# drprojects/superpoint_transformer

Hardware: AMD Instinct MI355X
Metric: Mpoints/s SPT fwd+bwd on S3DIS-scale NAG (higher is better)
Workload: dtype f32 (the reference's shipped matmul class - configs/train.yaml:60-61 `float32_matmul_precision: high` = TF32 / bf16x3 next to `precision: 32` - as bf16x3: matrix products on the bf16 pipe with split operands, attention and the backward of the fused layers and of the attention blocks' Linears hi*hi +

## Files before the change

superpoint_transformer_amd/csrc/fused_mlp.hip:

```cpp
#include <math.h>
#include <stdlib.h>

#include "common.hpp"

namespace spt {
namespace fmlp {

typedef float f32x4 __attribute__((ext_vector_type(4)));
constexpr int WAVES = 4;
constexpr int TR = 16;
constexpr int MAX_BLOCKS = 1024;
constexpr int MAX_BWD_WAVES = 4096;

__device__ __forceinline__ double xg_sum_d(double v) {
  v += __shfl_xor(v, 16, 64);
  v += __shfl_xor(v, 32, 64);
  return v;
}
__device__ __forceinline__ void wave_sync_lds() {
  __builtin_amdgcn_fence(__ATOMIC_RELEASE, "wavefront");
  __builtin_amdgcn_wave_barrier();
  __builtin_amdgcn_fence(__ATOMIC_ACQUIRE, "wavefront");
}

// ... 347 lines not shown
        *reinterpret_cast<float4*>(gl + rr * LDG + n) = v;
      }
    }
    stage_tile<KPP, LDX, KPP>(xprev, row0, cnt, K, false, pt, pslope, xl, nullptr, lane);
    wave_sync_lds();
#pragma unroll
    for (int r = 0; r < 4; ++r) {
      float xb[KB];
#pragma unroll
      for (int kb = 0; kb < KB; ++kb) {
        const int k = 16 * kb + c;
        float v = xl[(4 * g + r) * LDX + k];
        if (pre) {
          v = fmaf(v - pt[k], pt[KPP + k], pt[2 * KPP + k]);
          v = (v > 0.f) ? v : v * pslope;
          v = (4 * g + r < cnt && k < K) ? v : 0.f;
        }
        xb[kb] = v;
      }
#pragma unroll
      for (int nb = 0; nb < NBK; ++nb) {
        const float ga = gl[(4 * g + r) * LDG + 16 * nb + c];
#pragma unroll
        for (int kb = 0; kb < KB; ++kb)
          C3[nb][kb] = __builtin_amdgcn_mfma_f32_16x16x4f32(ga, xb[kb], C3[nb][kb], 0, 0, 0);
      }
    }
    if constexpr (NEED_GX) {
      f32x4 CX[KB];
#pragma unroll
      for (int kb = 0; kb < KB; ++kb) CX[kb] = (f32x4){0.f, 0.f, 0.f, 0.f};
      if constexpr (W_IN_LDS) {
        constexpr int G = (KB > 4) ? 1 : 2;
        float ac[G], bc[G][KB], an[G], bn[G][KB];
#pragma unroll
        for (int u = 0; u < G; ++u) {
          ac[u] = gl[c * LDG + 4 * u + g];
#pragma unroll
          for (int kb = 0; kb < KB; ++kb) bc[u][kb] = w_lds[(4 * u + g) * LDW + 16 * kb + c];
        }
#pragma unroll
        for (int grp = 0; grp < N / 4 / G; ++grp) {
          if (grp + 1 < N / 4 / G) {
#pragma unroll
            for (int u = 0; u < G; ++u) {
              const int st = G * (grp + 1) + u;
              an[u] = gl[c * LDG + 4 * st + g];
#pragma unroll
              for (int kb = 0; kb < KB; ++kb) bn[u][kb] = w_lds[(4 * st + g) * LDW + 16 * kb + c];
            }
          }
          __builtin_amdgcn_sched_barrier(0);
#pragma unroll
          for (int u = 0; u < G; ++u)
#pragma unroll
            for (int kb = 0; kb < KB; ++kb)
              CX[kb] = __builtin_amdgcn_mfma_f32_16x16x4f32(ac[u], bc[u][kb], CX[kb], 0, 0, 0);
          __builtin_amdgcn_sched_barrier(0);
#pragma unroll
          for (int u = 0; u < G; ++u) {
            ac[u] = an[u];
#pragma unroll
            for (int kb = 0; kb < KB; ++kb) bc[u][kb] = bn[u][kb];
          }
        }
      } else {
#pragma unroll
        for (int st = 0; st < N / 4; ++st) {
          const float a = gl[c * LDG + 4 * st + g];
#pragma unroll
          for (int kb = 0; kb < KB; ++kb)
            CX[kb] = __builtin_amdgcn_mfma_f32_16x16x4f32(a, BW[st][kb], CX[kb], 0, 0, 0);
        }
      }
#pragma unroll
      for (int r = 0; r < 4; ++r) {
        const int rr = 4 * g + r;
        if (rr < cnt) {
#pragma unroll
          for (int kb = 0; kb < KB; ++kb) {
            const int k = 16 * kb + c;
            if (k < K) {
              const float v = CX[kb][r];
              gx[(row0 + rr) * K + k] = v;
              if (pre) {
                const float o = xl[rr * LDX + k] - pt[k];
                float gg = v;
                if (pslope != 1.f) {
                  const float y = fmaf(o, pt[KPP + k], pt[2 * KPP + k]);
                  gg = (y > 0.f) ? gg : gg * pslope;
                }
                p1[kb] += (double)gg;
                p2[kb] += (double)gg * (double)o;
              }
            }
          }
        }
      }
    }
  }
  float* gwp = gw_partial + (size_t)wave * N * K;
#pragma unroll
  for (int nb = 0; nb < NBK; ++nb)
#pragma unroll
    for (int kb = 0; kb < KB; ++kb)
#pragma unroll
      for (int r = 0; r < 4; ++r) {
        const int k = 16 * kb + c;
        if (k < K) gwp[(size_t)(16 * nb + 4 * g + r) * K + k] = C3[nb][kb][r];
      }
  if (pstat_partial) {
    double* pp = pstat_partial + (size_t)wave * (2 * K + 1);
#pragma unroll
    for (int kb = 0; kb < KB; ++kb) {
      const double a = xg_sum_d(p1[kb]), b = xg_sum_d(p2[kb]);
      const int k = 16 * kb + c;
      if (g == 0 && k < K) {
        pp[k] = a;
        pp[K + k] = b;
      }
    }
    if (lane == 0) pp[2 * K] = (wave == 0) ? (double)(r1 - r0) : 0.0;
  }
}

typedef __bf16 bf16x8 __attribute__((ext_vector_type(8)));
typedef __bf16 bf16x4 __attribute__((ext_vector_type(4)));
typedef short s16x4 __attribute__((ext_vector_type(4)));

template <int NV, typename V>
__device__ __forceinline__ void split_bf16(const float (&x)[NV], V& hi, V& lo) {
#pragma unroll
  for (int i = 0; i < NV; ++i) {
    const __bf16 h = (__bf16)x[i];
    hi[i] = h;
    lo[i] = (__bf16)(x[i] - (float)h);
  }
}
template <bool LO>
__device__ __forceinline__ f32x4 mfma3_32(const bf16x8& ah, const bf16x8& al, const bf16x8& bh,
                                          const bf16x8& bl, f32x4 c) {
  if constexpr (LO) {
    c = __builtin_amdgcn_mfma_f32_16x16x32_bf16(al, bh, c, 0, 0, 0);
    c = __builtin_amdgcn_mfma_f32_16x16x32_bf16(ah, bl, c, 0, 0, 0);
  }
  return __builtin_amdgcn_mfma_f32_16x16x32_bf16(ah, bh, c, 0, 0, 0);
}
template <bool LO>
__device__ __forceinline__ f32x4 mfma3_16(const bf16x4& ah, const bf16x4& al, const bf16x4& bh,
                                          const bf16x4& bl, f32x4 c) {
  const s16x4 AH = __builtin_bit_cast(s16x4, ah), AL = __builtin_bit_cast(s16x4, al);
  const s16x4 BH = __builtin_bit_cast(s16x4, bh), BL = __builtin_bit_cast(s16x4, bl);
  if constexpr (LO) {
    c = __builtin_amdgcn_mfma_f32_16x16x16bf16_1k(AL, BH, c, 0, 0, 0);
    c = __builtin_amdgcn_mfma_f32_16x16x16bf16_1k(AH, BL, c, 0, 0, 0);
  }
  return __builtin_amdgcn_mfma_f32_16x16x16bf16_1k(AH, BH, c, 0, 0, 0);
}

template <int K4, int NBK, bool LO, bool IN16 = false, bool OUT16 = false>
__global__ __launch_bounds__(WAVES * 64, 2) void fwd_kernel_bf(
    const float* __restrict__ x, int64_t r0, int64_t r1, int K, const float* __restrict__ W,
    const float* __restrict__ am, const float* __restrict__ sc, const float* __restrict__ bs,
    float slope, float* __restrict__ h, double* __restrict__ partial, FmlpRuns rt) {
  constexpr int KP = K4 * 4, KS = (KP + 31) / 32, KP32 = KS * 32, LDA = KP32 + 4, N = NBK * 16;
  SPT_FMLP_RUN_FWD(N)
  __shared__ __attribute__((aligned(16))) float a_lds[WAVES][TR * LDA];
  __shared__ __attribute__((aligned(16))) float tab[3 * KP32];
  __shared__ double red[WAVES][2 * N];
  const int lane = threadIdx.x & 63;
  const int wid = __builtin_amdgcn_readfirstlane(threadIdx.x >> 6);
  const int g = lane >> 4, c = lane & 15;
  float* al = a_lds[wid];
  const bool pre = am != nullptr;
  load_table(tab, am, K, KP32);
  load_table(tab + KP32, sc, K, KP32);
  load_table(tab + 2 * KP32, bs, K, KP32);
  for (int i = lane; i < TR * LDA; i += 64) al[i] = 0.f;
  __syncthreads();

  bf16x8 Bh[NBK][KS], Bl[NBK][KS];
#pragma unroll
  for (int nb = 0; nb < NBK; ++nb)
#pragma unroll
    for (int ks = 0; ks < KS; ++ks) {
      float w[8];
#pragma unroll
      for (int i = 0; i < 8; ++i) {
        const int k = 32 * ks + 8 * g + i;
        w[i] = (k < K) ? W[(size_t)(16 * nb + c) * K + k] : 0.f;
      }
      split_bf16<8>(w, Bh[nb][ks], Bl[nb][ks]);
    }
  double s1[NBK], s2[NBK];
#pragma unroll
  for (int nb = 0; nb < NBK; ++nb) s1[nb] = s2[nb] = 0.0;

  const int64_t ntiles = (r1 - r0 + TR - 1) / TR;
  const int64_t wave = (int64_t)blockIdx.x * WAVES + wid;
  const int64_t nwaves = (int64_t)gridDim.x * WAVES;
  for (int64_t t = wave; t < ntiles; t += nwaves) {
    const int64_t row0 = r0 + t * TR;
    const int cnt = (int)((r1 - row0) < TR ? (r1 - row0) : TR);
    wave_sync_lds();
    stage_tile<KP32, LDA, KP32, false, 4, IN16>(x, row0, cnt, K, pre, tab, slope, al, nullptr, lane);
    wave_sync_lds();
    f32x4 C[NBK];
#pragma unroll
    for (int nb = 0; nb < NBK; ++nb) C[nb] = (f32x4){0.f, 0.f, 0.f, 0.f};
#pragma unroll
    for (int ks = 0; ks < KS; ++ks) {
      const float4 a0 = *reinterpret_cast<const float4*>(al + c * LDA + 32 * ks + 8 * g);
      const float4 a1 = *reinterpret_cast<const float4*>(al + c * LDA + 32 * ks + 8 * g + 4);
      const float av[8] = {a0.x, a0.y, a0.z, a0.w, a1.x, a1.y, a1.z, a1.w};
      bf16x8 ah, alo;
      split_bf16<8>(av, ah, alo);
#pragma unroll
      for (int nb = 0; nb < NBK; ++nb) C[nb] = mfma3_32<LO>(ah, alo, Bh[nb][ks], Bl[nb][ks], C[nb]);
    }
    if constexpr (OUT16) {
      constexpr int ROWB = 2 * N + 16;
      static_assert(TR * ROWB <= TR * LDA * 4, "the packed output tile fits the A-tile buffer");
      static_assert((TR * N / 8) % 64 == 0 || TR * N / 8 < 64, "whole 16-byte chunks");
      wave_sync_lds();
      char* ob = reinterpret_cast<char*>(al);
#pragma unroll
      for (int r = 0; r < 4; ++r) {
        const int rr = 4 * g + r;
#pragma unroll
        for (int nb = 0; nb < NBK; ++nb) {
          const unsigned mine = bf16_bits(C[nb][r]);
          const float vr = __uint_as_float(mine << 16);
          if (rr < cnt) {
            s1[nb] += (double)vr;
            s2[nb] += (double)vr * (double)vr;
          }
          const unsigned other = (unsigned)__builtin_amdgcn_update_dpp(0, (int)mine, 0xB1, 0xF, 0xF, false);
          if ((c & 1) == (r & 1)) {
            const unsigned w = (c & 1) ? (other | (mine << 16)) : (mine | (other << 16));
            *reinterpret_cast<unsigned*>(ob + rr * ROWB + (16 * nb + (c & ~1)) * 2) = w;
          }
        }
      }
      wave_sync_lds();
      constexpr int CPR = N / 8;
      uint16_t* h16 = reinterpret_cast<uint16_t*>(h);
#pragma unroll
      for (int q = lane; q < TR * CPR; q += 64) {
        const int rr = q / CPR, ch = q - rr * CPR;
        if (rr < cnt)
          *reinterpret_cast<uint4*>(h16 + (row0 + rr) * N + ch * 8) =
              *reinterpret_cast<const uint4*>(ob + rr * ROWB + ch * 16);
      }
    } else {
#pragma unroll
      for (int r = 0; r < 4; ++r) {
        const int rr = 4 * g + r;
        if (rr < cnt) {
          float* hr = h + (row0 + rr) * N + c;
#pragma unroll
          for (int nb = 0; nb < NBK; ++nb) {
            const float v = C[nb][r];
            hr[16 * nb] = v;
            s1[nb] += (double)v;
            s2[nb] += (double)v * (double)v;
          }
        }
      }
    }
  }
#pragma unroll
  for (int nb = 0; nb < NBK; ++nb) {
    const double a = xg_sum_d(s1[nb]), b = xg_sum_d(s2[nb]);
    if (g == 0) {
      red[wid][nb * 16 + c] = a;
      red[wid][N + nb * 16 + c] = b;
    }
  }
  __syncthreads();
  double* out = partial + (size_t)blockIdx.x * (2 * N + 1);
  for (int i = threadIdx.x; i < 2 * N; i += WAVES * 64)
    out[i] = ((red[0][i] + red[1][i]) + red[2][i]) + red[3][i];
  if (threadIdx.x == 0) out[2 * N] = (blockIdx.x == 0) ? (double)(r1 - r0) : 0.0;
}

constexpr int WAVES_X3 = 8;
template <int NV, typename V>
__device__ __forceinline__ void split3_bf16(const float (&x)[NV], V& h, V& m, V& l) {
#pragma unroll
  for (int i = 0; i < NV; ++i) {
    const __bf16 a = (__bf16)x[i];
    const float r1 = x[i] - (float)a;
    const __bf16 b = (__bf16)r1;
    const float r2 = r1 - (float)b;
    h[i] = a;
    m[i] = b;
    l[i] = (__bf16)r2;
  }
}
template <int K4, int NBK>
__global__ __launch_bounds__(WAVES_X3 * 64, 2) void fwd_kernel_x3(
    const float* __restrict__ x, int64_t r0, int64_t r1, int K, const float* __restrict__ W,
    const float* __restrict__ am, const float* __restrict__ sc, const float* __restrict__ bs,
    float slope, float* __restrict__ h, double* __restrict__ partial, FmlpRuns rt) {
  constexpr int KP = K4 * 4, KS = (KP + 31) / 32, KP32 = KS * 32, LDA = KP32 + 4, N = NBK * 16;
  constexpr int LDW = KP32 + 8;
  SPT_FMLP_RUN_FWD(N)
  __shared__ __attribute__((aligned(16))) float a_lds[WAVES_X3][TR * LDA];
// ... 1785 lines not shown
```

superpoint_transformer_amd/csrc/fused_mlp_dma.hip:

```cpp
#include <math.h>

#include "common.hpp"

#ifndef SPT_FDMA_SKIP
#define SPT_FDMA_SKIP 0
#endif

namespace spt {
namespace fdma {

typedef float f32x4 __attribute__((ext_vector_type(4)));
typedef __bf16 bf16x8 __attribute__((ext_vector_type(8)));
typedef __bf16 bf16x4 __attribute__((ext_vector_type(4)));
typedef short s16x4 __attribute__((ext_vector_type(4)));
constexpr int TR = 16;

__device__ __forceinline__ double xg_sum_d(double v) {
  v += __shfl_xor(v, 16, 64);
  v += __shfl_xor(v, 32, 64);
  return v;
}
__device__ __forceinline__ void lds_order() {
  __builtin_amdgcn_fence(__ATOMIC_RELEASE, "wavefront");
  __builtin_amdgcn_wave_barrier();
  __builtin_amdgcn_fence(__ATOMIC_ACQUIRE, "wavefront");
}
__device__ __forceinline__ void lds_dma16(const void* g, float* lds) {
#if SPT_FDMA_SKIP & 32
  return;
#endif
  const unsigned a = __builtin_amdgcn_readfirstlane(
      (unsigned)(size_t)((__attribute__((address_space(3))) void*)lds));
  asm volatile("s_mov_b32 m0, %0\n\ts_nop 0\n\tglobal_load_lds_dwordx4 %1, off"
               :: "s"(a), "v"(g) : "memory");
}
__device__ __forceinline__ void lds_dma4(const void* g, float* lds) {
#if SPT_FDMA_SKIP & 32
  return;
#endif
  const unsigned a = __builtin_amdgcn_readfirstlane(
      (unsigned)(size_t)((__attribute__((address_space(3))) void*)lds));
  asm volatile("s_mov_b32 m0, %0\n\ts_nop 0\n\tglobal_load_lds_dword %1, off"
               :: "s"(a), "v"(g) : "memory");
}
__device__ __forceinline__ void wait_vm0() {
  asm volatile("s_waitcnt vmcnt(0)" ::: "memory");
  __builtin_amdgcn_fence(__ATOMIC_ACQUIRE, "wavefront");
}
__device__ __forceinline__ void wait_lds() {
  asm volatile("s_waitcnt lgkmcnt(0)" ::: "memory");
}
__device__ __forceinline__ int opaque(int v) {
  asm volatile("" : "+v"(v));
  return v;
}
template <int NV, typename V>
__device__ __forceinline__ void split_bf16(const float (&x)[NV], V& hi, V& lo) {
#pragma unroll
  for (int i = 0; i < NV; ++i) {
    const __bf16 h = (__bf16)x[i];
    hi[i] = h;
    lo[i] = (__bf16)(x[i] - (float)h);
  }
}
template <bool LO>
__device__ __forceinline__ f32x4 mfma3_32(const bf16x8& ah, const bf16x8& al, const bf16x8& bh,
                                          const bf16x8& bl, f32x4 c) {
  if constexpr (LO) {
    c = __builtin_amdgcn_mfma_f32_16x16x32_bf16(al, bh, c, 0, 0, 0);
    c = __builtin_amdgcn_mfma_f32_16x16x32_bf16(ah, bl, c, 0, 0, 0);
  }
  return __builtin_amdgcn_mfma_f32_16x16x32_bf16(ah, bh, c, 0, 0, 0);
}
template <bool LO>
__device__ __forceinline__ f32x4 mfma3_16(const bf16x4& ah, const bf16x4& al, const bf16x4& bh,
                                          const bf16x4& bl, f32x4 c) {
  const s16x4 AH = __builtin_bit_cast(s16x4, ah), AL = __builtin_bit_cast(s16x4, al);
  const s16x4 BH = __builtin_bit_cast(s16x4, bh), BL = __builtin_bit_cast(s16x4, bl);
  if constexpr (LO) {
    c = __builtin_amdgcn_mfma_f32_16x16x16bf16_1k(AL, BH, c, 0, 0, 0);
    c = __builtin_amdgcn_mfma_f32_16x16x16bf16_1k(AH, BL, c, 0, 0, 0);
  }
  return __builtin_amdgcn_mfma_f32_16x16x16bf16_1k(AH, BH, c, 0, 0, 0);
}

template <int R>
__device__ __forceinline__ int pick_lane(int v, int base, int sel) {
  int r = __builtin_amdgcn_readlane(v, base);
#pragma unroll
  for (int j = 1; j < R; ++j) r = (sel == j) ? __builtin_amdgcn_readlane(v, base + j) : r;
  return r;
}

constexpr int fold_len(int K, int K0) { return (K + (K0 + 16) / 16 * 16) * ((K0 + 16) / 16 * 16); }
template <int K, int N, int NW, int OCC, bool LO, bool POOLED, bool S16 = false, int FK0 = 0>
__global__ __launch_bounds__(NW * 64, OCC) void bwd_dma_kernel(
    const float* __restrict__ gy, const float* __restrict__ h, int64_t r0, int64_t r1,
    const float* __restrict__ am, const float* __restrict__ sc, const float* __restrict__ bs,
    float slope, const float* __restrict__ c1, const float* __restrict__ c2,
    const float* __restrict__ c3, const float* __restrict__ xprev,
    const float* __restrict__ pam, const float* __restrict__ psc, const float* __restrict__ pbs,
    float pslope, const float* __restrict__ W, float* __restrict__ gx,
    float* __restrict__ gw_partial, double* __restrict__ pstat_partial,
    const int32_t* __restrict__ perm, const int32_t* __restrict__ pos_seg,
    const float* __restrict__ gout, const int32_t* __restrict__ arg, FmlpRuns rt,
    const float* __restrict__ x0 = nullptr, const float* __restrict__ fshift = nullptr,
    float* __restrict__ fold_partial = nullptr) {
  constexpr bool FOLD = FK0 > 0;
  constexpr int FOLD_K0 = FK0;
  static_assert(!FOLD || (!POOLED && !S16), "the fold reads dense f32 rows");
  constexpr int ZP = (FK0 + 16) / 16 * 16, ZB = ZP / 16;
  constexpr bool X0_DMA16 = FK0 % 4 == 0 && TR * FK0 * 4 <= 1024;
  constexpr int X0N = X0_DMA16 ? 1 : (TR * FK0 + 63) / 64;
  constexpr int X0LEN = X0_DMA16 ? 256 : 64 * X0N;
  static_assert(!FOLD || ZP <= 32, "the shift table holds 32 columns");
  constexpr int NC = N / 4, KC = K / 4, NBK = N / 16, KB = K / 16, NS = N / 32;
  if (rt.n > 0) {
    const int run_ = blockIdx.y, gph_ = rt.g[run_];
    r0 = rt.r0[run_];
    r1 = rt.r1[run_];
    am += (size_t)gph_ * N; sc += (size_t)gph_ * N;
    c1 += (size_t)gph_ * N; c2 += (size_t)gph_ * N; c3 += (size_t)gph_ * N;
    if (pam) { pam += (size_t)gph_ * K; psc += (size_t)gph_ * K; }
    gw_partial += (size_t)run_ * gridDim.x * N * K;
    if (pstat_partial) pstat_partial += (size_t)run_ * gridDim.x * NW * (2 * K + 1);
    if constexpr (FOLD) {
      fshift += (size_t)gph_ * 32;
      fold_partial += (size_t)run_ * gridDim.x * fold_len(K, FK0);
    }
  }
  constexpr int HI = TR * NC / 64, XI = TR * KC / 64;
  constexpr int RH = 64 / NC;
  constexpr int NSEG = RH;
  constexpr int LDT = N + 8;
  constexpr int W_H = TR * N, W_X = TR * K, W_G = POOLED ? NSEG * N : 0;
  static_assert(K % 16 == 0 && N % 32 == 0 && (TR * NC) % 64 == 0 && (TR * KC) % 64 == 0, "shape");
  __shared__ __attribute__((aligned(16))) float lw[NW][W_H + W_X + 2 * W_G];
  __shared__ __attribute__((aligned(16))) __bf16 wt_hi[K * LDT];
  __shared__ __attribute__((aligned(16))) __bf16 wt_lo[LO ? K * LDT : 8];
  __shared__ __attribute__((aligned(16))) float pt[3 * K];
  __shared__ __attribute__((aligned(16))) float x0b[FOLD ? NW : 1][FOLD ? X0LEN : 4];
  __shared__ float fsh[32];
  const int lane = threadIdx.x & 63;
  const int wid = __builtin_amdgcn_readfirstlane(threadIdx.x >> 6);
  const int g = lane >> 4, c = lane & 15;
  float* HB = lw[wid];
  float* XB = HB + W_H;
  float* GO = XB + W_X;
  int* AR = reinterpret_cast<int*>(GO + W_G);
  const bool pre = pam != nullptr;
  for (int i = threadIdx.x; i < K * N; i += NW * 64) {
    const int k = i / N, n = i - k * N;
    const float w = W[(size_t)n * K + k];
    const __bf16 hh = (__bf16)w;
    wt_hi[k * LDT + n] = hh;
    if constexpr (LO) wt_lo[k * LDT + n] = (__bf16)(w - (float)hh);
  }
  if constexpr (FOLD) {
    if (threadIdx.x < 32) fsh[threadIdx.x] = threadIdx.x < FOLD_K0 ? fshift[threadIdx.x] : 0.f;
  }
  for (int i = threadIdx.x; i < K; i += NW * 64) {
    pt[i] = pre ? pam[i] : 0.f;
    pt[K + i] = pre ? psc[i] : 1.f;
    pt[2 * K + i] = pre ? pbs[i] : 0.f;
  }
  __syncthreads();

  f32x4 C3[NBK][KB];
#pragma unroll
  for (int nb = 0; nb < NBK; ++nb)
#pragma unroll
    for (int kb = 0; kb < KB; ++kb) C3[nb][kb] = (f32x4){0.f, 0.f, 0.f, 0.f};
  double p1[KB], p2[KB];
#pragma unroll
  for (int kb = 0; kb < KB; ++kb) p1[kb] = p2[kb] = 0.0;
  f32x4 FA[FOLD ? KB : 1][ZB], FG[ZB][ZB];
#pragma unroll
  for (int zb = 0; zb < ZB; ++zb) {
#pragma unroll
    for (int kb = 0; kb < (FOLD ? KB : 1); ++kb) FA[kb][zb] = (f32x4){0.f, 0.f, 0.f, 0.f};
#pragma unroll
    for (int za = 0; za < ZB; ++za) FG[za][zb] = (f32x4){0.f, 0.f, 0.f, 0.f};
  }
  float* X0B = x0b[FOLD ? wid : 0];

  const int64_t ntiles = (r1 - r0 + TR - 1) / TR;
  const int64_t wave = (int64_t)blockIdx.x * NW + wid;
  const int64_t nwaves = (int64_t)gridDim.x * NW;

  const float4 t_am = *reinterpret_cast<const float4*>(am + 4 * (lane % NC));
  const float4 t_sc = *reinterpret_cast<const float4*>(sc + 4 * (lane % NC));
  const float4 t_bs = *reinterpret_cast<const float4*>(bs + 4 * (lane % NC));
  const float4 t_c1 = *reinterpret_cast<const float4*>(c1 + 4 * (lane % NC));
  const float4 t_c2 = *reinterpret_cast<const float4*>(c2 + 4 * (lane % NC));
  const float4 t_c3 = *reinterpret_cast<const float4*>(c3 + 4 * (lane % NC));
  int ln = opaque(lane);
  auto gh1 = [&](float hh, float gg, float aa, float ss, float bb, float q1, float q2, float q3) {
    const float o = hh - aa;
    if (slope != 1.f) {
      const float y = fmaf(o, ss, bb);
      gg = (y > 0.f) ? gg : gg * slope;
    }
    return fmaf(q1, gg, -fmaf(q2, o, q3));
  };
  auto gh_of = [&](const float4& hv, const float4& gv) {
    return make_float4(gh1(hv.x, gv.x, t_am.x, t_sc.x, t_bs.x, t_c1.x, t_c2.x, t_c3.x),
                       gh1(hv.y, gv.y, t_am.y, t_sc.y, t_bs.y, t_c1.y, t_c2.y, t_c3.y),
                       gh1(hv.z, gv.z, t_am.z, t_sc.z, t_bs.z, t_c1.z, t_c2.z, t_c3.z),
                       gh1(hv.w, gv.w, t_am.w, t_sc.w, t_bs.w, t_c1.w, t_c2.w, t_c3.w));
  };
  auto pick = [&](int v, int base) {
    const int hi = ln / NC;
    int r = __builtin_amdgcn_readlane(v, base);
#pragma unroll
    for (int j = 1; j < RH; ++j) r = (hi == j) ? __builtin_amdgcn_readlane(v, base + j) : r;
    return r;
  };
  constexpr int RX = 64 / KC;
  auto pickx = [&](int v, int base) {
    const int hx = ln / KC;
    int r = __builtin_amdgcn_readlane(v, base);
#pragma unroll
    for (int j = 1; j < RX; ++j) r = (hx == j) ? __builtin_amdgcn_readlane(v, base + j) : r;
    return r;
  };

  int rid_n = 0, seg_n = 0;
  auto load_ids = [&](int64_t t) {
    rid_n = seg_n = 0;
    const int64_t rowf = r0 + t * TR;
    if constexpr (POOLED) {
      if (t < ntiles && rowf + lane < r1 && lane < TR) {
        rid_n = perm[rowf + lane];
        seg_n = pos_seg[rowf + lane];
      }
    } else {
      if (t < ntiles && lane < TR) rid_n = (rowf + lane < r1) ? lane : 0;
    }
  };
  constexpr int NC16 = N / 8, RH16 = 64 / NC16, HI16 = TR / RH16;
  constexpr int KC16 = K / 8, RX16 = 64 / KC16, XI16 = (TR + RX16 - 1) / RX16;
  static_assert(!S16 || (TR % RH16 == 0 && RX16 <= TR), "bf16 rows: whole DMA instructions per tile");
  auto issue_h = [&](int64_t t, int rid_l, int seg_l) {
    if (t >= ntiles) return;
    const int64_t row0 = r0 + t * TR;
    const int hi = ln / NC, n4 = ln % NC;
    if constexpr (S16) {
      const uint16_t* hb = reinterpret_cast<const uint16_t*>(h) + (POOLED ? 0 : row0 * N);
      const int h16 = ln / NC16, p16 = ln % NC16;
#pragma unroll
      for (int i = 0; i < HI16; ++i)
        lds_dma16(hb + (int64_t)pick_lane<RH16>(rid_l, RH16 * i, h16) * N + 8 * p16,
                  HB + W_H / 2 + 256 * i);
    } else {
      const float* hb = POOLED ? h : h + row0 * N;
#pragma unroll
      for (int i = 0; i < HI; ++i) {
        const int rr7 = (hi + RH * i) & 7;
        lds_dma16(hb + (int64_t)pick(rid_l, RH * i) * N + 4 * (n4 ^ rr7), HB + 256 * i);
      }
    }
    if constexpr (POOLED) {
      const int cnt = (int)((r1 - row0) < TR ? (r1 - row0) : TR);
      const int s0 = __builtin_amdgcn_readlane(seg_l, 0);
      const int s1 = __builtin_amdgcn_readfirstlane(__shfl(seg_l, cnt - 1, 64));
      const int64_t sgm = (s0 + hi < s1) ? s0 + hi : s1;
      lds_dma16(gout + sgm * N + 4 * n4, GO);
      lds_dma16(arg + sgm * N + 4 * n4, reinterpret_cast<float*>(AR));
    }
  };
  auto issue_x = [&](int64_t t, int rid_l) {
    if (t >= ntiles) return;
    const int64_t row0 = r0 + t * TR;
    if constexpr (FOLD) {
      const int cnt = (int)((r1 - row0) < TR ? (r1 - row0) : TR);
      if constexpr (X0_DMA16) {
        const int last = cnt * FOLD_K0 - 4;
        lds_dma16(x0 + row0 * FOLD_K0 + (4 * ln < last ? 4 * ln : last), X0B);
      } else {
        const int last = cnt * FOLD_K0 - 1;
#pragma unroll
        for (int i = 0; i < X0N; ++i) {
          const int f = 64 * i + ln;
          lds_dma4(x0 + row0 * FOLD_K0 + (f < last ? f : last), X0B + 64 * i);
        }
      }
    }
    if constexpr (S16) {
      const uint16_t* xb = reinterpret_cast<const uint16_t*>(xprev) + (POOLED ? 0 : row0 * K);
      const int x16 = ln / KC16, q16 = ln % KC16;
#pragma unroll
      for (int i = 0; i < XI16; ++i)
        lds_dma16(xb + (int64_t)pick_lane<RX16>(rid_l, RX16 * i, x16) * K + 8 * q16,
                  XB + W_X / 2 + 256 * i);
    } else {
      const float* xb = POOLED ? xprev : xprev + row0 * K;
      const int hx = ln / KC, px = ln % KC;
#pragma unroll
      for (int i = 0; i < XI; ++i) {
        const int rr = hx + RX * i;
        lds_dma16(xb + (int64_t)pickx(rid_l, RX * i) * K + 4 * (px ^ (4 * ((rr >> 2) & 1))), XB + 256 * i);
      }
    }
  };

  load_ids(wave);
  int rid_l = rid_n, seg_l = seg_n;
  issue_h(wave, rid_l, seg_l);
  issue_x(wave, rid_l);
  load_ids(wave + nwaves);
  for (int64_t t = wave; t < ntiles; t += nwaves) {
    const int64_t row0 = r0 + t * TR;
    const int cnt = (int)((r1 - row0) < TR ? (r1 - row0) : TR);
    ln = opaque(ln);
    const int hi = ln / NC, n4 = ln % NC, hx = ln / KC, px = ln % KC, g = ln >> 4, c = ln & 15;
    float4 gyv[POOLED ? 1 : HI];
    if constexpr (!POOLED) {
#pragma unroll
      for (int i = 0; i < HI; ++i) {
        const int rr = hi + RH * i;
        gyv[i] = (rr < cnt) ? *reinterpret_cast<const float4*>(gy + (row0 + rr) * N + 4 * n4)
                            : make_float4(0.f, 0.f, 0.f, 0.f);
      }
    }
    wait_vm0();
    lds_order();
    if constexpr (S16) {
#pragma unroll
      for (int i = 0; i < XI; ++i) {
        const int rr = hx + RX * i;
        const int cx = px ^ (4 * ((rr >> 2) & 1));
        const uint2 u = *reinterpret_cast<const uint2*>(
            reinterpret_cast<const uint16_t*>(XB + W_X / 2) + rr * K + 4 * cx);
        *reinterpret_cast<float4*>(XB + rr * K + 4 * px) =
            make_float4(__uint_as_float(u.x << 16), __uint_as_float(u.x & 0xffff0000u),
                        __uint_as_float(u.y << 16), __uint_as_float(u.y & 0xffff0000u));
      }
    }
    if constexpr (!(SPT_FDMA_SKIP & 1)) {
      const int s0 = POOLED ? __builtin_amdgcn_readlane(seg_l, 0) : 0;
      const int s1 = POOLED ? __builtin_amdgcn_readfirstlane(__shfl(seg_l, cnt - 1, 64)) : 0;
      const bool in_lds = s1 - s0 < NSEG;
#pragma unroll
      for (int i = 0; i < HI; ++i) {
        const int rr = hi + RH * i;
        float* slot = HB + rr * N + 4 * (n4 ^ (rr & 7));
        float4 hv;
        if constexpr (S16) {
          const uint2 u = *reinterpret_cast<const uint2*>(
              reinterpret_cast<const uint16_t*>(HB + W_H / 2) + rr * N + 4 * n4);
          hv = make_float4(__uint_as_float(u.x << 16), __uint_as_float(u.x & 0xffff0000u),
                           __uint_as_float(u.y << 16), __uint_as_float(u.y & 0xffff0000u));
        } else {
          hv = *reinterpret_cast<const float4*>(slot);
        }
        float4 gv;
        if constexpr (POOLED) {
          const int rid = pick(rid_l, RH * i);
          const int sg = pick(seg_l, RH * i);
          int4 av;
          if (in_lds) {
            gv = *reinterpret_cast<const float4*>(GO + (sg - s0) * N + 4 * n4);
            av = *reinterpret_cast<const int4*>(AR + (sg - s0) * N + 4 * n4);
          } else {
            gv = *reinterpret_cast<const float4*>(gout + (int64_t)sg * N + 4 * n4);
            av = *reinterpret_cast<const int4*>(arg + (int64_t)sg * N + 4 * n4);
          }
          gv = make_float4(av.x == rid ? gv.x : 0.f, av.y == rid ? gv.y : 0.f,
                           av.z == rid ? gv.z : 0.f, av.w == rid ? gv.w : 0.f);
        } else {
          gv = gyv[i];
        }
        *reinterpret_cast<float4*>(slot) = gh_of(hv, gv);
      }
      if (cnt < TR) {
#pragma unroll
        for (int i = 0; i < HI; ++i) {
          const int rr = hi + RH * i;
          if (rr >= cnt)
            *reinterpret_cast<float4*>(HB + rr * N + 4 * (n4 ^ (rr & 7))) = make_float4(0.f, 0.f, 0.f, 0.f);
        }
      }
    }
    lds_order();
    if constexpr (!(SPT_FDMA_SKIP & 2)) {
      bf16x4 Xh[KB], Xl[KB];
#pragma unroll
      for (int kb = 0; kb < KB; ++kb) {
        const int k = 16 * kb + c;
        float xv[4];
#pragma unroll
        for (int r = 0; r < 4; ++r) {
          float v = XB[(4 * g + r) * K + 4 * ((4 * kb + (c >> 2)) ^ (4 * (g & 1))) + (c & 3)];
          if (pre) {
            v = fmaf(v - pt[k], pt[K + k], pt[2 * K + k]);
            v = (v > 0.f) ? v : v * pslope;
          }
          xv[r] = v;
        }
        split_bf16<4>(xv, Xh[kb], Xl[kb]);
      }
#pragma unroll
      for (int nb = 0; nb < NBK; ++nb) {
        float gv[4];
#pragma unroll
        for (int r = 0; r < 4; ++r)
          gv[r] = HB[(4 * g + r) * N + 4 * ((4 * nb + (c >> 2)) ^ (4 * (g & 1) + r)) + (c & 3)];
        bf16x4 gh4, gl4;
        split_bf16<4>(gv, gh4, gl4);
#pragma unroll
        for (int kb = 0; kb < KB; ++kb) C3[nb][kb] = mfma3_16<LO>(gh4, gl4, Xh[kb], Xl[kb], C3[nb][kb]);
      }
    }
    f32x4 CX[KB];
#pragma unroll
    for (int kb = 0; kb < KB; ++kb) CX[kb] = (f32x4){0.f, 0.f, 0.f, 0.f};
    if constexpr (!(SPT_FDMA_SKIP & 4)) {
#pragma unroll
      for (int sg = 0; sg < NS; ++sg) {
        const float4 a0 = *reinterpret_cast<const float4*>(HB + c * N + 4 * ((8 * sg + 2 * g) ^ (c & 7)));
        const float4 a1 = *reinterpret_cast<const float4*>(HB + c * N + 4 * ((8 * sg + 2 * g + 1) ^ (c & 7)));
        const float av[8] = {a0.x, a0.y, a0.z, a0.w, a1.x, a1.y, a1.z, a1.w};
        bf16x8 ah, alo;
        split_bf16<8>(av, ah, alo);
#pragma unroll
        for (int kb = 0; kb < KB; ++kb) {
          const bf16x8 bh = *reinterpret_cast<const bf16x8*>(wt_hi + (16 * kb + c) * LDT + 32 * sg + 8 * g);
          bf16x8 bl = bh;
          if constexpr (LO) bl = *reinterpret_cast<const bf16x8*>(wt_lo + (16 * kb + c) * LDT + 32 * sg + 8 * g);
          CX[kb] = mfma3_32<LO>(ah, alo, bh, bl, CX[kb]);
        }
      }
    }
    const int rid_cur = rid_l;
    wait_lds();
    issue_h(t + nwaves, rid_n, seg_n);
    bf16x4 X0h[ZB], X0l[ZB];
    if constexpr (FOLD) {
#pragma unroll
      for (int zb = 0; zb < ZB; ++zb) {
        const int col = 16 * zb + c;
        float x0v[4];
#pragma unroll
        for (int r = 0; r < 4; ++r) {
          const int rr = 4 * g + r;
          const float xr = X0B[rr * FOLD_K0 + (col < FOLD_K0 ? col : 0)];
          const float one = (col == FOLD_K0) ? 1.f : 0.f;
          x0v[r] = (rr < cnt) ? ((col < FOLD_K0) ? xr - fsh[col] : one) : 0.f;
        }
        split_bf16<4>(x0v, X0h[zb], X0l[zb]);
      }
#pragma unroll
      for (int za = 0; za < ZB; ++za)
#pragma unroll
        for (int zb = 0; zb < ZB; ++zb)
          FG[za][zb] = mfma3_16<LO>(X0h[za], X0l[za], X0h[zb], X0l[zb], FG[za][zb]);
    }
#pragma unroll
    for (int kb = 0; kb < KB; ++kb) {
      const int k = 16 * kb + c;
      float ggv[4] = {0.f, 0.f, 0.f, 0.f};
#pragma unroll
      for (int r = 0; r < 4; ++r) {
        float* xs = XB + (4 * g + r) * K + 4 * ((4 * kb + (c >> 2)) ^ (4 * (g & 1))) + (c & 3);
        const float v = CX[kb][r];
        if (!(SPT_FDMA_SKIP & 8) && pre) {
          const float o = *xs - pt[k];
          float gg = v;
          if (pslope != 1.f) {
            const float y = fmaf(o, pt[K + k], pt[2 * K + k]);
            gg = (y > 0.f) ? gg : gg * pslope;
          }
          p1[kb] += (double)gg;
          p2[kb] += (double)gg * (double)o;
          if constexpr (FOLD) ggv[r] = gg;
        }
        if constexpr (!FOLD) *xs = v;
      }
      if constexpr (FOLD) {
        bf16x4 ah, al;
        split_bf16<4>(ggv, ah, al);
#pragma unroll
        for (int zb = 0; zb < ZB; ++zb) FA[kb][zb] = mfma3_16<LO>(ah, al, X0h[zb], X0l[zb], FA[kb][zb]);
      }
    }
    if constexpr (!FOLD) {
      lds_order();
#pragma unroll
      for (int i = 0; i < XI; ++i) {
        const int rr = hx + RX * i;
        const float4 v = *reinterpret_cast<const float4*>(XB + rr * K + 4 * px);
        const int64_t orow = POOLED ? (int64_t)pickx(rid_cur, RX * i) : row0 + rr;
        if (!(SPT_FDMA_SKIP & 16) && rr < cnt)
          *reinterpret_cast<float4*>(gx + orow * K + 4 * (px ^ (4 * ((rr >> 2) & 1)))) = v;
      }
    }
    wait_lds();
    issue_x(t + nwaves, rid_n);
    rid_l = rid_n;
    seg_l = seg_n;
    load_ids(t + 2 * nwaves);
  }
  wait_vm0();
  {
    constexpr int LDR = K + 4;
    static_assert(N * LDR <= NW * (W_H + W_X + 2 * W_G), "the table fits the tile buffers");
    __syncthreads();
    float* red = &lw[0][0];
    for (int w = 1; w < NW; ++w) {
      if (wid == w) {
#pragma unroll
        for (int nb = 0; nb < NBK; ++nb)
#pragma unroll
          for (int kb = 0; kb < KB; ++kb)
#pragma unroll
            for (int r = 0; r < 4; ++r) red[(16 * nb + 4 * g + r) * LDR + 16 * kb + c] = C3[nb][kb][r];
      }
      __syncthreads();
      if (wid == 0) {
#pragma unroll
        for (int nb = 0; nb < NBK; ++nb)
#pragma unroll
          for (int kb = 0; kb < KB; ++kb)
#pragma unroll
            for (int r = 0; r < 4; ++r) C3[nb][kb][r] += red[(16 * nb + 4 * g + r) * LDR + 16 * kb + c];
      }
      __syncthreads();
    }
  }
  if (wid == 0) {
    float* gwp = gw_partial + (size_t)blockIdx.x * N * K;
#pragma unroll
    for (int nb = 0; nb < NBK; ++nb)
#pragma unroll
      for (int kb = 0; kb < KB; ++kb)
#pragma unroll
        for (int r = 0; r < 4; ++r)
          gwp[(size_t)(16 * nb + 4 * g + r) * K + 16 * kb + c] = C3[nb][kb][r];
  }
  if constexpr (FOLD) {
    constexpr int FLN = fold_len(K, FK0);
    static_assert(FLN <= NW * (W_H + W_X + 2 * W_G), "the fold table fits the tile buffers");
    float* red = &lw[0][0];
    for (int w = 1; w < NW; ++w) {
      if (wid == w) {
#pragma unroll
        for (int zb = 0; zb < ZB; ++zb)
#pragma unroll
          for (int r = 0; r < 4; ++r) {
#pragma unroll
            for (int kb = 0; kb < KB; ++kb) red[(16 * kb + 4 * g + r) * ZP + 16 * zb + c] = FA[kb][zb][r];
#pragma unroll
            for (int za = 0; za < ZB; ++za) red[(K + 16 * za + 4 * g + r) * ZP + 16 * zb + c] = FG[za][zb][r];
          }
      }
      __syncthreads();
      if (wid == 0) {
#pragma unroll
        for (int zb = 0; zb < ZB; ++zb)
#pragma unroll
          for (int r = 0; r < 4; ++r) {
#pragma unroll
            for (int kb = 0; kb < KB; ++kb) FA[kb][zb][r] += red[(16 * kb + 4 * g + r) * ZP + 16 * zb + c];
#pragma unroll
            for (int za = 0; za < ZB; ++za) FG[za][zb][r] += red[(K + 16 * za + 4 * g + r) * ZP + 16 * zb + c];
          }
      }
      __syncthreads();
    }
    if (wid == 0) {
      float* fp = fold_partial + (size_t)blockIdx.x * FLN;
#pragma unroll
      for (int zb = 0; zb < ZB; ++zb)
#pragma unroll
        for (int r = 0; r < 4; ++r) {
#pragma unroll
          for (int kb = 0; kb < KB; ++kb) fp[(16 * kb + 4 * g + r) * ZP + 16 * zb + c] = FA[kb][zb][r];
// ... 120 lines not shown
```

Measured before the change: 380.3.

## Store split bf16 gradient tile in LDS and read via transpose loads

The backward DMA kernel now splits the activation-gradient tile into bf16 hi/lo once when writing it, storing it in a swizzled bf16 LDS image. Both consumers then read it directly: the weight-gradient path uses ds_read_tr16_b64 transpose loads and the input-gradient path uses vector loads, so neither has to gather fp32 values and re-split them. Separately, the two cross-term 16x16x16 MFMAs in mfma3_16 are merged into one 16x16x32 MFMA on concatenated lo/hi operands, followed by an s_nop 15. That nop may add stall cycles, and the new swizzle has to stay correct for every N.

```diff
diff --git a/superpoint_transformer_amd/csrc/fused_mlp.hip b/superpoint_transformer_amd/csrc/fused_mlp.hip
--- a/superpoint_transformer_amd/csrc/fused_mlp.hip
+++ b/superpoint_transformer_amd/csrc/fused_mlp.hip
@@ -523,8 +523,10 @@
   const s16x4 AH = __builtin_bit_cast(s16x4, ah), AL = __builtin_bit_cast(s16x4, al);
   const s16x4 BH = __builtin_bit_cast(s16x4, bh), BL = __builtin_bit_cast(s16x4, bl);
   if constexpr (LO) {
-    c = __builtin_amdgcn_mfma_f32_16x16x16bf16_1k(AL, BH, c, 0, 0, 0);
-    c = __builtin_amdgcn_mfma_f32_16x16x16bf16_1k(AH, BL, c, 0, 0, 0);
+    const bf16x8 A = __builtin_bit_cast(bf16x8, __builtin_shufflevector(AL, AH, 0, 1, 2, 3, 4, 5, 6, 7));
+    const bf16x8 B = __builtin_bit_cast(bf16x8, __builtin_shufflevector(BH, BL, 0, 1, 2, 3, 4, 5, 6, 7));
+    c = __builtin_amdgcn_mfma_f32_16x16x32_bf16(A, B, c, 0, 0, 0);
+    asm volatile("s_nop 15" : "+v"(c));
   }
   return __builtin_amdgcn_mfma_f32_16x16x16bf16_1k(AH, BH, c, 0, 0, 0);
 }
diff --git a/superpoint_transformer_amd/csrc/fused_mlp_dma.hip b/superpoint_transformer_amd/csrc/fused_mlp_dma.hip
--- a/superpoint_transformer_amd/csrc/fused_mlp_dma.hip
+++ b/superpoint_transformer_amd/csrc/fused_mlp_dma.hip
@@ -78,8 +78,10 @@
   const s16x4 AH = __builtin_bit_cast(s16x4, ah), AL = __builtin_bit_cast(s16x4, al);
   const s16x4 BH = __builtin_bit_cast(s16x4, bh), BL = __builtin_bit_cast(s16x4, bl);
   if constexpr (LO) {
-    c = __builtin_amdgcn_mfma_f32_16x16x16bf16_1k(AL, BH, c, 0, 0, 0);
-    c = __builtin_amdgcn_mfma_f32_16x16x16bf16_1k(AH, BL, c, 0, 0, 0);
+    const bf16x8 A = __builtin_bit_cast(bf16x8, __builtin_shufflevector(AL, AH, 0, 1, 2, 3, 4, 5, 6, 7));
+    const bf16x8 B = __builtin_bit_cast(bf16x8, __builtin_shufflevector(BH, BL, 0, 1, 2, 3, 4, 5, 6, 7));
+    c = __builtin_amdgcn_mfma_f32_16x16x32_bf16(A, B, c, 0, 0, 0);
+    asm volatile("s_nop 15" : "+v"(c));
   }
   return __builtin_amdgcn_mfma_f32_16x16x16bf16_1k(AH, BH, c, 0, 0, 0);
 }
@@ -90,6 +92,19 @@
 #pragma unroll
   for (int j = 1; j < R; ++j) r = (sel == j) ? __builtin_amdgcn_readlane(v, base + j) : r;
   return r;
+}
+
+template <int N>
+__device__ __forceinline__ int gp_off(int row, int col) {
+  constexpr int RPL = N >= 64 ? 1 : 64 / N;
+  static_assert(N == 32 || N == 64 || N == 128, "image row of 128, 256 or 512 bytes");
+  const int swz = ((row / RPL) & (8 / RPL - 1)) << 1;
+  return row * 2 * N + ((((col >> 3) ^ swz) << 3) | (col & 7));
+}
+typedef __attribute__((address_space(3))) s16x4 lds_s16x4;
+__device__ __forceinline__ bf16x4 tr_read(const __bf16* p) {
+  return __builtin_bit_cast(bf16x4, __builtin_amdgcn_ds_read_tr16_b64_v4i16(
+                                        (lds_s16x4*)(__attribute__((address_space(3))) void*)p));
 }
 
 constexpr int fold_len(int K, int K0) { return (K + (K0 + 16) / 16 * 16) * ((K0 + 16) / 16 * 16); }
@@ -145,6 +160,7 @@
   const int wid = __builtin_amdgcn_readfirstlane(threadIdx.x >> 6);
   const int g = lane >> 4, c = lane & 15;
   float* HB = lw[wid];
+  __bf16* GP = reinterpret_cast<__bf16*>(HB);
   float* XB = HB + W_H;
   float* GO = XB + W_X;
   int* AR = reinterpret_cast<int*>(GO + W_G);
@@ -344,7 +360,6 @@
 #pragma unroll
       for (int i = 0; i < HI; ++i) {
         const int rr = hi + RH * i;
-        float* slot = HB + rr * N + 4 * (n4 ^ (rr & 7));
         float4 hv;
         if constexpr (S16) {
           const uint2 u = *reinterpret_cast<const uint2*>(
@@ -352,7 +367,7 @@
           hv = make_float4(__uint_as_float(u.x << 16), __uint_as_float(u.x & 0xffff0000u),
                            __uint_as_float(u.y << 16), __uint_as_float(u.y & 0xffff0000u));
         } else {
-          hv = *reinterpret_cast<const float4*>(slot);
+          hv = *reinterpret_cast<const float4*>(HB + rr * N + 4 * (n4 ^ (rr & 7)));
         }
         float4 gv;
         if constexpr (POOLED) {
@@ -371,14 +386,22 @@
         } else {
           gv = gyv[i];
         }
-        *reinterpret_cast<float4*>(slot) = gh_of(hv, gv);
+        const float4 q = gh_of(hv, gv);
+        const float qv[4] = {q.x, q.y, q.z, q.w};
+        bf16x4 qh, ql;
+        split_bf16<4>(qv, qh, ql);
+        *reinterpret_cast<bf16x4*>(GP + gp_off<N>(rr, 4 * n4)) = qh;
+        if constexpr (LO) *reinterpret_cast<bf16x4*>(GP + gp_off<N>(rr, N + 4 * n4)) = ql;
       }
       if (cnt < TR) {
+        const bf16x4 z = __builtin_bit_cast(bf16x4, make_uint2(0u, 0u));
 #pragma unroll
         for (int i = 0; i < HI; ++i) {
           const int rr = hi + RH * i;
-          if (rr >= cnt)
-            *reinterpret_cast<float4*>(HB + rr * N + 4 * (n4 ^ (rr & 7))) = make_float4(0.f, 0.f, 0.f, 0.f);
+          if (rr >= cnt) {
+            *reinterpret_cast<bf16x4*>(GP + gp_off<N>(rr, 4 * n4)) = z;
+            if constexpr (LO) *reinterpret_cast<bf16x4*>(GP + gp_off<N>(rr, N + 4 * n4)) = z;
+          }
         }
       }
     }
@@ -400,14 +423,12 @@
         }
         split_bf16<4>(xv, Xh[kb], Xl[kb]);
       }
+      const int trow = 4 * g + (c >> 2), tcol = 4 * (c & 3);
 #pragma unroll
       for (int nb = 0; nb < NBK; ++nb) {
-        float gv[4];
-#pragma unroll
-        for (int r = 0; r < 4; ++r)
-          gv[r] = HB[(4 * g + r) * N + 4 * ((4 * nb + (c >> 2)) ^ (4 * (g & 1) + r)) + (c & 3)];
-        bf16x4 gh4, gl4;
-        split_bf16<4>(gv, gh4, gl4);
+        const bf16x4 gh4 = tr_read(GP + gp_off<N>(trow, 16 * nb + tcol));
+        bf16x4 gl4 = gh4;
+        if constexpr (LO) gl4 = tr_read(GP + gp_off<N>(trow, N + 16 * nb + tcol));
 #pragma unroll
         for (int kb = 0; kb < KB; ++kb) C3[nb][kb] = mfma3_16<LO>(gh4, gl4, Xh[kb], Xl[kb], C3[nb][kb]);
       }
@@ -418,11 +439,9 @@
     if constexpr (!(SPT_FDMA_SKIP & 4)) {
 #pragma unroll
       for (int sg = 0; sg < NS; ++sg) {
-        const float4 a0 = *reinterpret_cast<const float4*>(HB + c * N + 4 * ((8 * sg + 2 * g) ^ (c & 7)));
-        const float4 a1 = *reinterpret_cast<const float4*>(HB + c * N + 4 * ((8 * sg + 2 * g + 1) ^ (c & 7)));
-        const float av[8] = {a0.x, a0.y, a0.z, a0.w, a1.x, a1.y, a1.z, a1.w};
-        bf16x8 ah, alo;
-        split_bf16<8>(av, ah, alo);
+        const bf16x8 ah = *reinterpret_cast<const bf16x8*>(GP + gp_off<N>(c, 32 * sg + 8 * g));
+        bf16x8 alo = ah;
+        if constexpr (LO) alo = *reinterpret_cast<const bf16x8*>(GP + gp_off<N>(c, N + 32 * sg + 8 * g));
 #pragma unroll
         for (int kb = 0; kb < KB; ++kb) {
           const bf16x8 bh = *reinterpret_cast<const bf16x8*>(wt_hi + (16 * kb + c) * LDT + 32 * sg + 8 * g);
```

Result: no change. 380.0 (-0.1%).
